# qqueing/DeepSpeaker-pytorch

Measured on AMD Instinct MI355X. Metric: embeddings/sec (64-fbank x 160-frame utterances), higher is better.
Workload: dtype f16

## Files before the change

### deepspeaker-pytorch_amd/_native.py

```python
from __future__ import annotations

import ctypes
import os
from ctypes import POINTER, Structure, c_char_p, c_double, c_float, c_int, c_longlong, c_void_p

_HERE = os.path.dirname(os.path.abspath(__file__))
LIB_NAME = "libdeepspeaker_hip.so"

DS_EPI_AFFINE, DS_EPI_RESIDUAL, DS_EPI_CLIP, DS_EPI_STATS, DS_EPI_OUT_F32, DS_EPI_OUT_F16 = 1, 2, 4, 8, 16, 32
DS_EPI_OUT_PLANES16, DS_CONV_IN_PLANES16 = 256, 512
DS_CONV_HINT_SINGLE_BUFFER = 64
DS_CONV_HINT_CHUNK16 = 128
DS_CONV_HINT_NO_PERSIST = 1024
DS_CONV_HINT_NO_WIDE = 2048
DS_CONV_HINT_ONE_QUEUE = 4096
DS_CONV_PLAN_LATENCY = 8192
DS_CONV_CK = 8
DS_TAIL_SMALL_MAX_B = 4
DS_MARGIN_AAM, DS_MARGIN_AM = 0, 1
DS_MARGIN_SIN2_FLOOR = 1e-6


class ConvShape(Structure):
    _fields_ = [("B", c_int), ("H", c_int), ("W", c_int), ("Cin", c_int),
# ... 19 lines not shown
    "ds_event_elapsed_ms": (c_int, [_P, _P, POINTER(c_float)]),
    "ds_launch_timing_arm": (c_int, [_P, _P]),
    "ds_launch_timing_end": (c_int, []),
    "ds_error_string": (c_char_p, [c_int]),
    "ds_sched_workspace_bytes": (ctypes.c_size_t, []),
    "ds_sched_set_workspace": (c_int, [_P, ctypes.c_size_t]),
    "ds_sched_free_slots": (c_longlong, []),
    "ds_nchw_to_nhwc_f32": (c_int, [_P, _P, c_int, c_int, c_int, c_int, _P]),
    "ds_nhwc_to_nchw_f32": (c_int, [_P, _P, c_int, c_int, c_int, c_int, _P]),
    "ds_pack_conv_weight_f32": (c_int, [_P, _P, c_int, c_int, c_int, c_int, _P]),
    "ds_pack_conv1_weight_f32": (c_int, [_P, _P, c_int, _P]),
    "ds_pack_fc_weight_f32": (c_int, [_P, _P, c_int, c_int, c_int, _P]),
    "ds_pack_fc_weight_dgrad_f32": (c_int, [_P, _P, c_int, c_int, c_int, _P]),
    "ds_bn_fold_f32": (c_int, [_P, _P, _P, _P, c_float, _P, _P, c_int, _P]),
    "ds_bn_stats_finalize_f32": (c_int, [_P, c_int, c_longlong, _P, _P, c_float, c_float, _P, _P, _P, _P,
                                         _P, _P, c_int, _P]),
    "ds_bn_apply_f32": (c_int, [_P, _P, _P, _P, _P, c_longlong, c_int, c_int, _P]),
    "ds_conv_out_dims": (c_int, [POINTER(ConvShape), POINTER(c_int), POINTER(c_int)]),
    "ds_conv_stats_rows": (c_int, [POINTER(ConvShape)]),
    "ds_conv_plan_describe": (c_int, [POINTER(ConvShape), POINTER(c_int)]),
    "ds_conv_f32_set_forced_cfg": (None, [c_int]),
    "ds_conv5x5s2_c1_stats_rows": (c_int, [c_int, c_int]),
    "ds_conv5x5s2_c1_fwd_f32": (c_int, [_P, _P, _P, _P, _P, _P, c_int, c_int, c_int, c_int, c_int, _P]),
    "ds_conv5x5s2_c1_fwd_bf16": (c_int, [_P, _P, _P, _P, _P, _P, c_int, c_int, c_int, c_int, c_int, _P]),
    "ds_conv_fwd_f32": (c_int, [POINTER(ConvShape), _P, _P, _P, _P, _P, _P, _P, c_int, _P]),
    "ds_pack_conv_weight_bf16": (c_int, [_P, _P, _P, c_int, c_int, c_int, _P]),
    "ds_pack_conv_weight_dgrad_bf16": (c_int, [_P, _P, _P, c_int, c_int, c_int, _P]),
    "ds_pack_conv_weight_dgrad_s2_bf16": (c_int, [_P, _P, _P, c_int, c_int, _P]),
    "ds_conv_dgrad_bf16": (c_int, [POINTER(ConvShape), _P, _P, _P, _P, _P]),
    "ds_conv_bf16_stats_rows": (c_int, [POINTER(ConvShape), c_int]),
    "ds_conv_bf16_plan_describe": (c_int, [POINTER(ConvShape), c_int, POINTER(c_int)]),
    "ds_conv_bf16_plan_describe_hinted": (c_int, [POINTER(ConvShape), c_int, c_int, POINTER(c_int)]),
    "ds_conv_bf16_set_forced_cfg": (None, [c_int]),
    "ds_conv_fwd_bf16": (c_int, [POINTER(ConvShape), _P, _P, _P, _P, _P, _P, _P, _P, c_int, _P]),
    "ds_pack_conv_weight_f16": (c_int, [_P, _P, c_int, c_int, c_int, _P]),
    "ds_pack_conv_weights_f16_batch": (c_int, [POINTER(PackJob), c_int, _P]),
    "ds_pack_conv_weights_bf16_batch": (c_int, [POINTER(PackJob), c_int, _P]),
    "ds_conv_fwd_f16": (c_int, [POINTER(ConvShape), _P, _P, _P, _P, _P, _P, c_int, _P]),
    "ds_conv_f16_splitk_workspace_bytes": (c_longlong, [POINTER(ConvShape)]),
    "ds_conv_fwd_f16_splitk": (c_int, [POINTER(ConvShape), _P, _P, _P, _P, _P, _P, c_int, _P, c_longlong, _P]),
    "ds_conv_block_f16_supported": (c_int, [c_int, c_int, c_int, c_int]),
    "ds_conv_block_f16": (c_int, [_P, _P, _P, _P, _P, _P, _P, _P, c_int, c_int, c_int, c_int, c_int, _P]),
    "ds_conv_block_f16_masked": (c_int, [_P, _P, _P, _P, _P, _P, _P, _P, _P, c_int, c_int, c_int, c_int, c_int, _P]),
    "ds_conv_f16_plan_describe": (c_int, [POINTER(ConvShape), POINTER(c_int)]),
    "ds_conv_f16_plan_describe_hinted": (c_int, [POINTER(ConvShape), c_int, POINTER(c_int)]),
    "ds_conv_f16_set_layout_padding": (None, [c_int]),
    "ds_conv_f16_set_forced_cfg": (None, [c_int]),
    "ds_conv_f16_plan_lds_layout": (c_int, [POINTER(ConvShape), c_int, POINTER(c_int)]),
    "ds_cast_f32_to_f16": (c_int, [_P, _P, c_longlong, _P]),
    "ds_cast_f16_to_f32": (c_int, [_P, _P, c_longlong, _P]),
    "ds_avgpool_time_f32": (c_int, [_P, _P, c_int, c_int, c_int, c_int, _P]),
    "ds_l2norm_scale_f32": (c_int, [_P, _P, c_int, c_int, c_float, c_float, _P]),
    "ds_max_abs_diff_f32": (c_int, [_P, _P, c_longlong, _P, _P]),
    "ds_fc_workspace_floats": (c_longlong, [c_int, c_int, c_int]),
    "ds_fc_l2norm_fwd_f32": (c_int, [_P, _P, _P, _P, _P, _P, c_int, c_int, c_int, c_float, c_float, _P]),
    "ds_pairwise_distance_f32": (c_int, [_P, _P, _P, c_int, c_int, _P]),
    "ds_pairwise_distance_p_f32": (c_int, [_P, _P, _P, c_int, c_int, c_float, _P]),
    "ds_pairwise_distance_p_bwd_f32": (c_int, [_P, _P, _P, _P, _P, _P, c_int, c_int, c_float, _P]),
    "ds_triplet_margin_fwd_f32": (c_int, [_P, _P, _P, c_float, _P, _P, _P, c_int, c_int, _P]),
    "ds_triplet_filter_f32": (c_int, [_P, _P, c_float, _P, _P, _P, c_int, _P]),
    "ds_triplet_tail_f32": (c_int, [_P, _P, _P, c_float, c_float, _P, _P, _P, _P, _P, _P, _P, _P, c_int, c_int, c_int, _P]),
    "ds_triplet_scan_f32": (c_int, [_P, _P, c_float, _P, _P, _P, _P, c_int, _P]),
    "ds_refine_distances_f32": (c_int, [_P, _P, _P, c_int, _P, _P, c_int, _P]),
    "ds_triplet_tail_probe_f32": (c_int, [_P, _P, _P, c_float, c_float, _P, _P, _P, _P, _P, _P, _P, _P, c_int, c_int, c_int,
                                          c_int, _P]),
    "ds_refine_distances_probe_f32": (c_int, [_P, _P, _P, c_int, _P, _P, _P, _P, _P, _P, _P, c_int, _P, _P]),
# ... 226 lines not shown
```

### deepspeaker-pytorch_amd/csrc/conv_mfma_bf16.hip

```cpp
#include <ds_device.h>
#include <algorithm>
#include "ds_common.h"

#include "conv_mfma_bf16_kernel.h"
#include "conv_plan.h"

namespace {

__device__ __forceinline__ void pack_conv_weight_bf16_body(const float *w, __bf16 *hi, __bf16 *lo, int Cout, int Cin, int KS,
                                                           int dgrad, int block, int n_blocks) {
    const int T = KS * KS;
    const long long n = (long long)Cout * Cin * T;
    const int N = dgrad ? Cin : Cout;
    for (long long i = (long long)block * 256 + threadIdx.x; i < n; i += (long long)n_blocks * 256) {
        const int kk = (int)(i & 15);
        long long r = i >> 4;
        const int nn = (int)(r % N);
        r /= N;
        const int t = (int)(r % T);
        const int kc = (int)(r / T);
        const int k = kc * 16 + kk;
        const int tt = dgrad ? (T - 1 - t) : t;
        const int kh = tt / KS, kw = tt - kh * KS;
        const int co = dgrad ? k : nn, ci = dgrad ? nn : k;
// ... 18 lines not shown
};

__global__ void __launch_bounds__(256) pack_conv_weight_bf16_batch_kernel(const PackBatchB J) {
    int j = 0;
    while (j + 1 < J.n && (int)blockIdx.x >= J.first[j + 1]) ++j;
    pack_conv_weight_bf16_body(J.w[j], J.hi[j], J.lo[j], J.Cout[j], J.Cin[j], J.KS[j], J.dgrad[j], (int)blockIdx.x - J.first[j],
                               J.first[j + 1] - J.first[j]);
}

static double frag_read_cost(int MT, int NI, int RT, int Wc, int IS, int rows_in, int pitch) {
    const int pix_per_seg = RT * Wc, seg_pix = rows_in * pitch;
    double total = 0.0;
    int n = 0;
    for (int m0 = 0; m0 + 32 <= MT; m0 += 32) {
        for (int g = 0; g < 2; ++g) {
            int cnt[16] = {0};
            int worst = 0;
            for (int j = 0; j < 16; ++j) {
                const int m = m0 + 16 * g + j;
                const int seg = m / pix_per_seg, rem = m % pix_per_seg;
                const int r = rem / Wc, c = rem % Wc;
                const int rec = (seg < NI) ? seg * seg_pix + (IS * r) * pitch + c : 0;
                const int slot = (rec * (PSB / 16)) & 15;
                if (++cnt[slot] > worst) worst = cnt[slot];
            }
            total += worst;
            ++n;
        }
    }
    return n ? total / n : 1.0;
}

static int g_forced_cfg_b = -1;

constexpr int kPlanLatRows = 1;
constexpr int kPlanLatency = 2;

constexpr size_t kLdsSlackB = 16;
static size_t plan_lds_bytes(const TileCfgB &cf, size_t tile_pix, bool x3, int NI) {
    return std::max(tile_pix * PSB * (x3 ? 2 : 1), cf.epi_bytes()) + (size_t)cf.MT() * 4 + (size_t)NI * 8 + (size_t)cf.WM * cf.NTILE() * 8;
}

static int plan_bf16(PlanB &pl, const ds_conv_shape *s, bool x3, int out_stride = 1, int out_h0 = 0, int out_w0 = 0,
                     int out_H = 0, int out_W = 0, int grid_H = 0, int grid_W = 0, int mode = 0) {
    int Ho, Wo;
    const int rc = ds_plan_check_shape(s, CKB, false, Ho, Wo, grid_H, grid_W);
    if (rc != DS_OK) return rc;
    const int pad = s->KS / 2;
    const int yH = out_H > 0 ? out_H : Ho, yW = out_W > 0 ? out_W : Wo;
    DS_REQUIRE((long long)s->B * Ho < (1ll << 24), DS_ERR_BAD_SHAPE);
    DS_REQUIRE((long long)s->B * yH * yW * s->Cout < (1ll << 30), DS_ERR_BAD_SHAPE);
    const int IS = s->stride;
    double best = -1.0;
    int bc = -1, brt = 0, bni = 0;
    long long bwaves = 0, bcost = 0, bblocks = 0;
    bool latency = false;
    auto search = [&](int c) {
        const TileCfgB &cf = ds_bf16_cfg(c);
        if (s->Cout % cf.NTILE()) return;
        if (cf.x3_only && !x3) return;
        if (g_forced_cfg_b >= 0 && c != g_forced_cfg_b) return;
        const long long item_cap = (long long)cf.items_per_thread * cf.NTHR();
        auto fits = [&](int n, int rows_in, int cols_in) {
            return plan_lds_bytes(cf, (size_t)n * rows_in * (cols_in + 4), x3, n) <= cf.lds_cap &&
                   (long long)n * std::min(rows_in, s->H) * s->W * (CKB / 4) <= item_cap;
        };
        ds_plan_segmentations(s->B, Ho, Wo, cf.MT(), IS, s->KS, s->KS, fits, [&](int rt, int ni, long long n_mt) {
            const long long blocks = n_mt * (s->Cout / cf.NTILE());
            double eff = ds_plan_fill_occupancy(s->B, Ho, Wo, n_mt, cf.MT(), blocks, cf.wg_per_cu);
            const long long waves = blocks * (cf.NTHR() / 64);
            if (waves < kPlanSIMDs) eff *= (double)waves / (double)kPlanSIMDs;
            int pref[kNumCfgBAll] = {0, 2, 7, 8, 5, 6, 1, 4, 3, 0, 0};
#ifdef DS_BF16_PREF_TOP
            pref[DS_BF16_PREF_TOP] = 9;
#endif
            eff += 1e-9 * rt + 1e-6 * pref[c];
            bool better = eff > best;
            const long long cost = ds_ceil_div_ll(waves, kPlanSIMDs) * ((x3 ? 3 : 1) * cf.MSUB * cf.NSUB);
            if (latency && bc >= 0) {
                const TileCfgB &bf = ds_bf16_cfg(bc);
                const int area = cf.MT() * cf.NTILE(), barea = bf.MT() * bf.NTILE();
                if (cost != bcost) better = cost < bcost;
                else if (area != barea) better = area > barea;
                else if (blocks != bblocks) better = blocks < bblocks;
            }
            if (better) { best = eff; bc = c; brt = rt; bni = ni; bwaves = waves; bcost = cost; bblocks = blocks; }
        });
    };
    const bool forced_lat = (mode & kPlanLatRows) && g_forced_cfg_b >= kNumCfgB;
    for (int c = 0; c < (forced_lat ? kNumCfgBAll : kNumCfgB); ++c) search(c);
    if ((mode & kPlanLatency) && x3 && g_forced_cfg_b < 0 && bc >= 0 && bwaves < kPlanSIMDs) {
        latency = true;
        best = -1.0;
        bc = -1;
        for (int c = 0; c < kNumCfgBAll; ++c) search(c);
    }
    if (bc < 0) return DS_ERR_UNSUPPORTED;
    const TileCfgB &cf = ds_bf16_cfg(bc);
    ConvKB &k = pl.k;
    k.H = s->H; k.W = s->W; k.Cin = s->Cin;
    k.Hr = Ho; k.Wc = Wo; k.Ho = yH; k.Wo = yW; k.Cout = s->Cout;
    k.OS = out_stride; k.OH0 = out_h0; k.OW0 = out_w0;
    k.IS = IS; k.dh_min = -pad; k.dw_min = -pad;
    pl.cfg = bc;
    ds_plan_fill_geometry(pl, s->B, Ho, Wo, IS, s->KS, s->KS, s->Cout, cf.NTILE(), brt, bni);
    k.half = (k.cols_in + 1) / 2;
    int best_pitch = k.cols_in;
    double best_cost = 1e30;
    for (int pt = k.cols_in; pt <= k.cols_in + 4; ++pt) {
        const double c = frag_read_cost(cf.MT(), bni, brt, Wo, IS, k.rows_in, pt);
        if (c < best_cost - 1e-9) { best_cost = c; best_pitch = pt; }
    }
    k.pitch = best_pitch;
    k.seg_pix = k.rows_in * k.pitch;
    k.y_bytes = (unsigned)((long long)s->B * yH * yW * s->Cout * 4);
    pl.lds_bytes = plan_lds_bytes(cf, (size_t)k.NI * k.seg_pix, x3, k.NI) + kLdsSlackB;
    pl.nit = ds_ceil_div(k.NI * std::min(k.rows_in, s->H) * s->W * (CKB / 4), cf.NTHR());
    k.bn_z = k.bn_mean = k.bn_invstd = k.bn_msc = k.bn_msh = nullptr;
    k.bn_mtiles = 1; k.bn_rows_member = 0; k.bn_row0 = 0;
    return DS_OK;
}

static void set_operands(ConvKB &k, const float *x, const void *w_hi, const void *w_lo, float *y, const float *scale,
                         const float *shift, const float *res, float *stats, int flags) {
    k.x = x; k.w_hi = (const __bf16 *)w_hi; k.w_lo = (const __bf16 *)w_lo; k.y = y;
    k.scale = scale; k.shift = shift; k.res = res; k.stats = stats;
    k.flags = flags;
}

template <int KS, bool X3>
static void launch_b(const PlanB &pl, void *stream) {
    if (pl.cfg >= kNumCfgB) {
        if (KS == 3) ds_bf16_launch_k3x3l(pl, stream); else ds_bf16_launch_k5x3l(pl, stream);
        return;
    }
    if (KS == 3) { if (X3) ds_bf16_launch_k3x3(pl, stream); else ds_bf16_launch_k3x1(pl, stream); }
    else         { if (X3) ds_bf16_launch_k5x3(pl, stream); else ds_bf16_launch_k5x1(pl, stream); }
}

}

static int pack_job_check(const void *w_oihw, const void *w_hi, int Cout, int Cin, int KS, int dgrad, int bad_ks, long long *n) {
    DS_REQUIRE(w_oihw && w_hi, DS_ERR_NULL);
    DS_REQUIRE((dgrad == 0 || dgrad == 1) && Cout > 0 && Cin > 0, DS_ERR_BAD_SHAPE);
    DS_REQUIRE(KS == 3 || KS == 5, bad_ks);
    DS_REQUIRE((dgrad ? Cout : Cin) % CKB == 0, DS_ERR_BAD_SHAPE);
    *n = (long long)Cout * Cin * KS * KS;
    return DS_OK;
}

static int pack_bf16(const float *w_oihw, void *w_hi, void *w_lo, int Cout, int Cin, int KS, int dgrad, void *stream) {
    long long n;
    const int rc = pack_job_check(w_oihw, w_hi, Cout, Cin, KS, dgrad, DS_ERR_BAD_SHAPE, &n);
    if (rc != DS_OK) return rc;
    long long g = (n + 255) / 256;
    DS_LAUNCH(pack_conv_weight_bf16_kernel, (int)(g > 4096 ? 4096 : g), 256, 0, stream, w_oihw, (__bf16 *)w_hi,
              (__bf16 *)w_lo, Cout, Cin, KS, dgrad);
    return ds_last_launch_error();
}

extern "C" int ds_pack_conv_weights_bf16_batch(const ds_pack_job *jobs, int n_jobs, void *stream) {
    DS_REQUIRE(jobs != nullptr, DS_ERR_NULL);
    DS_REQUIRE(n_jobs > 0 && n_jobs <= DS_PACK_BATCH_MAX, DS_ERR_BAD_SHAPE);
    PackBatchB J;
// ... 4 lines not shown
        long long n;
        const int rc = pack_job_check(b.w_oihw, b.out, b.Cout, b.Cin, b.KS, b.mode, DS_ERR_UNSUPPORTED, &n);
        if (rc != DS_OK) return rc;
        J.w[j] = b.w_oihw; J.hi[j] = (__bf16 *)b.out; J.lo[j] = (__bf16 *)b.out2;
        J.Cout[j] = b.Cout; J.Cin[j] = b.Cin; J.KS[j] = b.KS; J.dgrad[j] = b.mode;
        const long long g = (n + 255) / 256;
        J.first[j] = blocks;
        blocks += (int)(g > 512 ? 512 : g);
    }
    J.first[n_jobs] = blocks;
    DS_LAUNCH(pack_conv_weight_bf16_batch_kernel, blocks, 256, 0, stream, J);
    return ds_last_launch_error();
}

extern "C" int ds_pack_conv_weight_bf16(const float *w_oihw, void *w_hi, void *w_lo, int Cout, int Cin, int KS,
                                        void *stream) {
    return pack_bf16(w_oihw, w_hi, w_lo, Cout, Cin, KS, 0, stream);
}

extern "C" int ds_pack_conv_weight_dgrad_bf16(const float *w_oihw, void *w_hi, void *w_lo, int Cout, int Cin, int KS,
                                              void *stream) {
    return pack_bf16(w_oihw, w_hi, w_lo, Cout, Cin, KS, 1, stream);
}

static int fwd_plan_mode(int flags) { return kPlanLatRows | ((flags & DS_CONV_PLAN_LATENCY) ? kPlanLatency : 0); }

extern "C" int ds_conv_bf16_stats_rows(const ds_conv_shape *s, int x3) {
    PlanB pl;
    int rc = plan_bf16(pl, s, x3 != 0, 1, 0, 0, 0, 0, 0, 0, fwd_plan_mode(0));
    return rc == DS_OK ? pl.n_mtiles : rc;
}

extern "C" void ds_conv_bf16_set_forced_cfg(int cfg) { g_forced_cfg_b = (cfg >= 0 && cfg < kNumCfgBAll) ? cfg : -1; }

extern "C" int ds_conv_bf16_plan_describe(const ds_conv_shape *s, int x3, int *out8) {
    return ds_conv_bf16_plan_describe_hinted(s, x3, 0, out8);
}

extern "C" int ds_conv_bf16_plan_describe_hinted(const ds_conv_shape *s, int x3, int flags, int *out8) {
    DS_REQUIRE(out8 != nullptr, DS_ERR_NULL);
    PlanB pl;
    int rc = plan_bf16(pl, s, x3 != 0, 1, 0, 0, 0, 0, 0, 0, fwd_plan_mode(flags));
    if (rc != DS_OK) return rc;
    const TileCfgB &cf = ds_bf16_cfg(pl.cfg);
    out8[0] = cf.MT(); out8[1] = cf.NTILE(); out8[2] = pl.k.RT; out8[3] = pl.k.NI;
    out8[4] = pl.grid; out8[5] = (int)pl.lds_bytes; out8[6] = cf.NTHR(); out8[7] = pl.k.pitch;
    return DS_OK;
}

extern "C" int ds_conv_fwd_bf16(const ds_conv_shape *s, const float *x, const void *w_hi, const void *w_lo,
                                const float *scale, const float *shift, const float *residual, float *y,
                                float *stats_partial, int flags, void *stream) {
    DS_REQUIRE(x && w_hi && y, DS_ERR_NULL);
    DS_REQUIRE(!(flags & DS_EPI_AFFINE) || (scale && shift), DS_ERR_NULL);
    DS_REQUIRE(!(flags & DS_EPI_RESIDUAL) || residual, DS_ERR_NULL);
    DS_REQUIRE(!(flags & DS_EPI_STATS) || stats_partial, DS_ERR_NULL);
    DS_REQUIRE(!((flags & DS_CONV_PLAN_LATENCY) && (flags & DS_EPI_STATS)), DS_ERR_UNSUPPORTED);
    DS_REQUIRE(DS_ALIGNED16(x) && DS_ALIGNED16(w_hi) && DS_ALIGNED16(y) && DS_ALIGNED16(w_lo), DS_ERR_ALIGNMENT);
    const bool x3 = w_lo != nullptr;
    PlanB pl;
    int rc = plan_bf16(pl, s, x3, 1, 0, 0, 0, 0, 0, 0, fwd_plan_mode(flags));
    if (rc != DS_OK) return rc;
    set_operands(pl.k, x, w_hi, w_lo, y, scale, shift, residual, stats_partial, flags & ~DS_CONV_PLAN_LATENCY);
    if (s->KS == 3) { if (x3) launch_b<3, true>(pl, stream); else launch_b<3, false>(pl, stream); }
    else            { if (x3) launch_b<5, true>(pl, stream); else launch_b<5, false>(pl, stream); }
    return ds_last_launch_error();
// ... 176 lines not shown
```

### deepspeaker-pytorch_amd/csrc/conv_mfma_bf16_kernel.h

```cpp
#pragma once
#include <ds_device.h>
#include <type_traits>
#include "ds_common.h"
#include "conv_mfma_f16_parts.h"


constexpr int CKB = 16;
constexpr int PSB = 48;


struct ConvKB {
    const float *x;
    const __bf16 *w_hi, *w_lo;
    float *y;
    const float *scale, *shift, *res;
    float *stats;
    int H, W, Cin;
    int Hr, Wc, Ho, Wo, Cout;
    int IS;
    int dh_min, dw_min;
    int rows_in, cols_in, seg_pix;
    int pitch, half;
    int RT, NI, segs_per_img, n_segs;
    int n_ntiles;
    int flags;
    unsigned y_bytes;
    int OS, OH0, OW0;
    const float *bn_z, *bn_mean, *bn_invstd, *bn_msc, *bn_msh;
    int bn_mtiles;
    int bn_rows_member, bn_row0;
};

struct PlanB {
    int cfg, grid, n_mtiles, nit;
    size_t lds_bytes;
    ConvKB k;
};

struct TileCfgB {
    int MSUB, NSUB, WM, WN;
    int wg_per_cu;
    size_t lds_cap;
    int items_per_thread;
    bool x3_only;
    constexpr int MT() const { return MSUB * WM * 32; }
    constexpr int NTILE() const { return NSUB * WN * 32; }
    constexpr int NTHR() const { return WM * WN * 64; }
    constexpr size_t epi_bytes() const { return (size_t)WM * WN * 32 * (NSUB * 32 + 4) * 4; }
};
constexpr int kNumCfgB = 9;
constexpr TileCfgB kCfgB[kNumCfgB] = {
    {2, 1, 2, 2, 3, 64 * 1024, 16, false},
    {5, 1, 1, 4, 2, 64 * 1024, 16, false},
    {4, 1, 2, 2, 2, 64 * 1024, 16, false},
    {5, 2, 1, 2, 2, 80 * 1024, 32, true},
    {5, 2, 1, 4, 1, 160 * 1024 - 64, 32, true},
    {5, 2, 2, 2, 1, 160 * 1024 - 64, 32, true},
    {5, 2, 2, 1, 2, 80 * 1024, 32, true},
    {4, 2, 1, 2, 2, 80 * 1024, 32, true},
    {4, 2, 1, 4, 1, 160 * 1024 - 64, 32, true},
};

constexpr int kNumCfgBLat = 2;
constexpr TileCfgB kCfgBLat[kNumCfgBLat] = {
    {1, 1, 2, 2, 2, 64 * 1024, 16, true},
    {1, 1, 1, 4, 2, 64 * 1024, 16, true},
};
constexpr int kNumCfgBAll = kNumCfgB + kNumCfgBLat;
constexpr const TileCfgB &ds_bf16_cfg(int cfg) { return cfg < kNumCfgB ? kCfgB[cfg] : kCfgBLat[cfg - kNumCfgB]; }

void ds_bf16_launch_k3x3(const PlanB &pl, void *stream);
void ds_bf16_launch_k5x3(const PlanB &pl, void *stream);
void ds_bf16_launch_k3x1(const PlanB &pl, void *stream);
void ds_bf16_launch_k5x1(const PlanB &pl, void *stream);
void ds_bf16_launch_k3x3g(const PlanB &pl, void *stream);
void ds_bf16_launch_k3x3l(const PlanB &pl, void *stream);
void ds_bf16_launch_k5x3l(const PlanB &pl, void *stream);

#ifdef DS_BF16_KERNEL_TU
namespace {

template <int KS, int MSUB, int NSUB, int WM, int WN, bool X3, int NIT, bool PREF, bool BNB = false>
__global__ void __launch_bounds__(WM * WN * 64) conv_mfma_bf16_kernel(const ConvKB p) {
    constexpr int NTHR = WM * WN * 64;
    constexpr int MT = MSUB * WM * 32;
    constexpr int NTILE = NSUB * WN * 32;
    constexpr int NT = KS * KS;
    constexpr int RING = (KS == 3) ? (MSUB <= 2 ? 9 : 3) : (KS == 5 ? 5 : 1);
    constexpr bool APREF = (MSUB * NSUB >= 8);
    constexpr bool ILV = X3 && APREF;

    char *lds = (char *)ds_dynamic_lds();
    const int tid = threadIdx.x, lane = tid & 63, wave = tid >> 6;
    const int wm = wave / WN, wn = wave % WN;
    const int l31 = lane & 31, lhi = lane >> 5;
    const int tile_n = blockIdx.x % p.n_ntiles;
    const int tile_m = blockIdx.x / p.n_ntiles;
    const int seg0 = tile_m * p.NI;
    const int pix_per_seg = p.RT * p.Wc;
    const int tile_pix = p.NI * p.seg_pix;
    constexpr int EPI_BYTES = WM * WN * 32 * (NSUB * 32 + 4) * 4;
    const int tile_bytes = (X3 ? 2 : 1) * tile_pix * PSB;
    const int stage_bytes = tile_bytes > EPI_BYTES ? tile_bytes : EPI_BYTES;
    char *lds_hi = lds;
    char *lds_lo = lds + (X3 ? tile_pix * PSB : 0);
    int *out_off = (int *)(lds + stage_bytes);
    int *seg_lo = out_off + MT;
    int *seg_cnt = seg_lo + p.NI;
    float *red = (float *)(seg_cnt + p.NI);

    const int n_chunks = p.Cin / CKB;
    const int n_base = tile_n * NTILE + wn * NSUB * 32;
    const size_t lane_w = ((size_t)(n_base + l31) * CKB + 8 * lhi);
    const size_t w_tap_stride = (size_t)p.Cout * CKB;
    const int last_tap = n_chunks * NT - 1;

    bf16x8 bq_hi[RING][NSUB], bq_lo[X3 ? RING : 1][NSUB];
#pragma unroll
    for (int d = 0; d < RING; ++d)
#pragma unroll
        for (int ns = 0; ns < NSUB; ++ns) {
            const int g = d < last_tap ? d : last_tap;
            const size_t o = lane_w + (size_t)g * w_tap_stride + (size_t)ns * 32 * CKB;
            bq_hi[d][ns] = *(const bf16x8 *)(p.w_hi + o);
            if constexpr (X3) bq_lo[d][ns] = *(const bf16x8 *)(p.w_lo + o);
        }

    const float rcp_pps = 1.0f / (float)pix_per_seg, rcp_wc = 1.0f / (float)p.Wc, rcp_w = 1.0f / (float)p.W,
                rcp_spi = 1.0f / (float)p.segs_per_img;
    for (int seg = tid; seg < p.NI; seg += NTHR) {
        const int gseg = seg0 + seg;
        int lo = 0, cnt = 0;
        if (gseg < p.n_segs) {
            const int b = ds_div_small(gseg, p.segs_per_img, rcp_spi);
            const int h0 = p.IS * (gseg - b * p.segs_per_img) * p.RT + p.dh_min;
            lo = h0 < 0 ? -h0 : 0;
// ... 28 lines not shown
                cnt = seg_cnt[seg];
                lo = seg_lo[seg];
                const int gseg = seg0 + seg;
                const int b = ds_div_small(gseg, p.segs_per_img, rcp_spi);
                img_row = b * p.H + p.IS * (gseg - b * p.segs_per_img) * p.RT + p.dh_min;
            }
        };
        next_seg();
#pragma unroll
        for (int it = 0; it < NIT; ++it) {
            while (seg < p.NI && vr >= row0 + cnt) next_seg();
            g_off[it] = 0;
            l_off[it] = 32;
            if (seg < p.NI) {
                const int rr = lo + vr - row0;
                const int cc = c - p.dw_min;
                const int pc = (p.IS == 2) ? ((cc & 1) ? p.half + (cc >> 1) : (cc >> 1)) : cc;
                g_off[it] = ((img_row + rr) * p.W + c) * p.Cin + q * 4;
                l_off[it] = (seg * p.seg_pix + rr * p.pitch + pc) * PSB + q * 8;
            }
            c += dc;
            vr += dvr;
            if (c >= p.W) {
                c -= p.W;
                ++vr;
            }
        }
    }
    f32x4 st[NIT];
    if constexpr (PREF) {
#pragma unroll
        for (int it = 0; it < NIT; ++it) st[it] = *(const f32x4 *)(p.x + g_off[it]);
    }
    for (int i = tid; i < tile_bytes / 16; i += NTHR) *(f32x4 *)(lds + 16 * i) = f32x4{0.0f, 0.0f, 0.0f, 0.0f};
    for (int m = tid; m < MT; m += NTHR) {
        const int seg = ds_div_small(m, pix_per_seg, rcp_pps);
        const int rem = m - seg * pix_per_seg;
        const int r = ds_div_small(rem, p.Wc, rcp_wc), c = rem - r * p.Wc;
        const int gseg = seg0 + seg;
        int off = -1;
        if (seg < p.NI && gseg < p.n_segs) {
            const int b = ds_div_small(gseg, p.segs_per_img, rcp_spi);
            const int rr = (gseg - b * p.segs_per_img) * p.RT + r;
            if (rr < p.Hr) off = ((b * p.Ho + p.OS * rr + p.OH0) * p.Wo + p.OS * c + p.OW0) * p.Cout;
        }
        out_off[m] = off;
    }
    const int lpix = ds_mfma_lpix(l31);
    int a_off[MSUB];
#pragma unroll
    for (int ms = 0; ms < MSUB; ++ms) {
        const int m = (wm * MSUB + ms) * 32 + lpix;
        const int seg = ds_div_small(m, pix_per_seg, rcp_pps);
        const int rem = m - seg * pix_per_seg;
        const int r = ds_div_small(rem, p.Wc, rcp_wc), c = rem - r * p.Wc;
        const int pix = (seg < p.NI) ? seg * p.seg_pix + (p.IS * r) * p.pitch + c : 0;
        a_off[ms] = pix * PSB + 16 * lhi;
    }

    constexpr bool CVI = ILV && PREF;
    constexpr int CV_FIRST = 3;
    auto split_item = [&](int it) {
        const f32x4 v = st[it];
        bf16x8 pk;
#pragma unroll
        for (int j = 0; j < 4; ++j) {
            const __bf16 h = (__bf16)v[j];
            pk[j] = h;
            pk[4 + j] = (__bf16)(v[j] - (float)h);
        }
        st[it] = __builtin_bit_cast(f32x4, pk);
    };
    if constexpr (CVI) {
#pragma unroll
        for (int it = 0; it < NIT; ++it) split_item(it);
    }

    for (int chunk = 0; chunk < n_chunks; ++chunk) {
        __syncthreads();
        if constexpr (!PREF) {
#pragma unroll
            for (int it = 0; it < NIT; ++it) st[it] = *(const f32x4 *)(p.x + g_off[it] + chunk * CKB);
        }
        if constexpr (CVI) {
#pragma unroll
            for (int it = 0; it < NIT; ++it) {
                const bf16x8 pk = __builtin_bit_cast(bf16x8, st[it]);
                *(bf16x4 *)(lds_hi + l_off[it]) = __builtin_shufflevector(pk, pk, 0, 1, 2, 3);
                *(bf16x4 *)(lds_lo + l_off[it]) = __builtin_shufflevector(pk, pk, 4, 5, 6, 7);
            }
        } else {
#pragma unroll
            for (int it = 0; it < NIT; ++it) {
                const f32x4 v = st[it];
                bf16x4 h;
#pragma unroll
                for (int j = 0; j < 4; ++j) h[j] = (__bf16)v[j];
                *(bf16x4 *)(lds_hi + l_off[it]) = h;
                if constexpr (X3) {
                    bf16x4 l;
#pragma unroll
                    for (int j = 0; j < 4; ++j) l[j] = (__bf16)(v[j] - (float)h[j]);
                    *(bf16x4 *)(lds_lo + l_off[it]) = l;
                }
            }
        }
        __syncthreads();
        if constexpr (PREF) {
            const int cn = chunk + 1 < n_chunks ? chunk + 1 : chunk;
#pragma unroll
// ... 271 lines not shown
    else if (pl.nit <= 16)
        DS_LAUNCH_BIG_LDS((conv_mfma_bf16_kernel<KS, MSUB, NSUB, WM, WN, true, 16, true, BNB>), pl.grid, NTHR, pl.lds_bytes, stream, pl.k);
    else
        DS_LAUNCH_BIG_LDS((conv_mfma_bf16_kernel<KS, MSUB, NSUB, WM, WN, true, 32, false, BNB>), pl.grid, NTHR, pl.lds_bytes, stream, pl.k);
}

template <int N = 0, class F>
static void ds_bf16_with_cfg(int cfg, F &&f) {
    if constexpr (N < kNumCfgB) {
        if (cfg == N) f(std::integral_constant<int, N>{});
        else ds_bf16_with_cfg<N + 1>(cfg, f);
    }
}

template <int KS, bool X3, bool BNB = false>
static void launch_b(const PlanB &pl, void *stream) {
    ds_bf16_with_cfg(pl.cfg, [&](auto c) {
        constexpr TileCfgB cf = kCfgB[decltype(c)::value];
        if constexpr (!cf.x3_only) launch_nit_b<KS, cf.MSUB, cf.NSUB, cf.WM, cf.WN, X3, BNB>(pl, stream);
        else if constexpr (X3) launch_big_b<KS, cf.MSUB, cf.NSUB, cf.WM, cf.WN, BNB>(pl, stream);
    });
}

template <int KS, int N = 0>
static void launch_lat_b(const PlanB &pl, void *stream) {
    if constexpr (N < kNumCfgBLat) {
        constexpr TileCfgB cf = kCfgBLat[N];
        static_assert(cf.NTHR() == 256, "launch_nit_b launches 256 threads");
        if (pl.cfg - kNumCfgB == N) launch_nit_b<KS, cf.MSUB, cf.NSUB, cf.WM, cf.WN, true>(pl, stream);
        else launch_lat_b<KS, N + 1>(pl, stream);
    }
}

}
#endif
```

### include/deepspeaker_hip.h

```cpp
#ifndef DEEPSPEAKER_HIP_H
#define DEEPSPEAKER_HIP_H

#include <stddef.h>
#include <stdint.h>

#ifdef __cplusplus
extern "C" {
#endif

#define DS_OK               0
#define DS_ERR_BAD_SHAPE   (-1)
#define DS_ERR_ALIGNMENT   (-2)
#define DS_ERR_NULL        (-3)
#define DS_ERR_UNSUPPORTED (-4)
#define DS_ERR_NO_WORKSPACE (-5)

#define DS_EPI_AFFINE   1
#define DS_EPI_RESIDUAL 2
#define DS_EPI_CLIP     4
#define DS_EPI_STATS    8

#define DS_EPI_OUT_F32  16
#define DS_EPI_OUT_F16  32

// ... 54 lines not shown
    int B, H, W, Cin;
    int Cout, KS;
    int stride;
} ds_conv_shape;

int ds_conv_out_dims(const ds_conv_shape *s, int *Ho, int *Wo);
int ds_conv_stats_rows(const ds_conv_shape *s);

int ds_conv_plan_describe(const ds_conv_shape *s, int *out8);
void ds_conv_f32_set_forced_cfg(int cfg);
int ds_conv5x5s2_c1_stats_rows(int B, int H);
int ds_conv5x5s2_c1_fwd_f32(const float *x, const float *w_packed, const float *scale,
                            const float *shift, float *y, float *stats_partial, int B, int H,
                            int W, int Cout, int flags, void *stream);
int ds_conv5x5s2_c1_fwd_bf16(const float *x, const float *w_packed, const float *scale,
                             const float *shift, void *y, float *stats_partial, int B, int H,
                             int W, int Cout, int flags, void *stream);
int ds_conv_fwd_f32(const ds_conv_shape *s, const float *x, const float *w_packed,
                    const float *scale, const float *shift, const float *residual, float *y,
                    float *stats_partial, int flags, void *stream);

int ds_pack_conv_weight_bf16(const float *w_oihw, void *w_hi, void *w_lo, int Cout, int Cin, int KS,
                             void *stream);
int ds_pack_conv_weight_dgrad_bf16(const float *w_oihw, void *w_hi, void *w_lo, int Cout, int Cin,
                                   int KS, void *stream);
int ds_pack_conv_weight_dgrad_s2_bf16(const float *w_oihw, void *w_hi, void *w_lo, int Cout, int Cin,
                                      void *stream);
int ds_conv_dgrad_bf16(const ds_conv_shape *s, const float *gy, const void *w_hi, const void *w_lo,
                       float *gx, void *stream);
int ds_conv_bf16_stats_rows(const ds_conv_shape *s, int x3);
int ds_conv_bf16_plan_describe(const ds_conv_shape *s, int x3, int *out8);
int ds_conv_bf16_plan_describe_hinted(const ds_conv_shape *s, int x3, int flags, int *out8);
void ds_conv_bf16_set_forced_cfg(int cfg);
int ds_conv_fwd_bf16(const ds_conv_shape *s, const float *x, const void *w_hi, const void *w_lo,
                     const float *scale, const float *shift, const float *residual, float *y,
                     float *stats_partial, int flags, void *stream);

int ds_pack_conv_weight_f16(const float *w_oihw, void *w_f16, int Cout, int Cin, int KS, void *stream);
int ds_conv_fwd_f16(const ds_conv_shape *s, const void *x_f16, const void *w_f16, const float *scale,
                    const float *shift, const void *residual_f16, void *y, int flags, void *stream);
long long ds_conv_f16_splitk_workspace_bytes(const ds_conv_shape *s);
int ds_conv_fwd_f16_splitk(const ds_conv_shape *s, const void *x_f16, const void *w_f16, const float *scale,
                           const float *shift, const void *residual_f16, void *y, int flags, void *workspace,
                           long long ws_bytes, void *stream);
int ds_conv_f16_plan_describe(const ds_conv_shape *s, int *out8);
int ds_conv_f16_plan_describe_hinted(const ds_conv_shape *s, int flags, int *out8);
int ds_conv_f16_plan_lds_layout(const ds_conv_shape *s, int flags, int *out4);
void ds_conv_f16_set_layout_padding(int on);
void ds_conv_f16_set_forced_cfg(int cfg);
int ds_conv_block_f16_supported(int B, int H, int W, int C);
int ds_conv_block_f16(const void *x_f16, const void *wa_f16, const void *wb_f16, const float *scale_a,
                      const float *shift_a, const float *scale_b, const float *shift_b, void *y, int B, int H, int W,
                      int C, int flags, void *stream);
int ds_conv_block_f16_masked(const void *x_f16, const void *wa_f16, const void *wb_f16, const float *scale_a,
                             const float *shift_a, const float *scale_b, const float *shift_b, void *y, const int *lens,
                             int B, int H, int W, int C, int flags, void *stream);
int ds_cast_f32_to_f16(const float *x, void *y_f16, long long n, void *stream);
int ds_cast_f16_to_f32(const void *x_f16, float *y, long long n, void *stream);

int ds_avgpool_time_f32(const float *x, float *pooled, int B, int Hr, int Wc, int C, void *stream);
int ds_l2norm_scale_f32(const float *f, float *e, int B, int D, float alpha, float eps,
                        void *stream);

int ds_max_abs_diff_f32(const float *a, const float *b, long long n, float *out2, void *stream);

long long ds_fc_workspace_floats(int B, int K, int N);
// ... 257 lines not shown
```

Before: 401,200.

## Add double-buffered pipelined bf16x3 conv walk for sub-chip latency plans

Adds a PIPE variant of the bf16x3 MFMA conv kernel that double-buffers the input tile in LDS and interleaves the global load and hi/lo split of the next chunk with the MFMAs of the current chunk. Weight fragments are prefetched through a ring. The planner picks this path for latency-mode x3 plans that occupy less than the chip, when the doubled LDS still fits. The cost is double LDS per block and more template instantiations. This only touches the bf16 x3 path, while the workload is f16 inference, so it likely does not run in the benchmark.

```diff
diff --git a/deepspeaker-pytorch_amd/_native.py b/deepspeaker-pytorch_amd/_native.py
--- a/deepspeaker-pytorch_amd/_native.py
+++ b/deepspeaker-pytorch_amd/_native.py
@@ -75,6 +75,8 @@
     "ds_conv_bf16_plan_describe": (c_int, [POINTER(ConvShape), c_int, POINTER(c_int)]),
     "ds_conv_bf16_plan_describe_hinted": (c_int, [POINTER(ConvShape), c_int, c_int, POINTER(c_int)]),
     "ds_conv_bf16_set_forced_cfg": (None, [c_int]),
+    "ds_conv_bf16_set_walk": (None, [c_int]),
+    "ds_conv_bf16_plan_walk": (c_int, [POINTER(ConvShape), c_int, c_int]),
     "ds_conv_fwd_bf16": (c_int, [POINTER(ConvShape), _P, _P, _P, _P, _P, _P, _P, _P, c_int, _P]),
     "ds_pack_conv_weight_f16": (c_int, [_P, _P, c_int, c_int, c_int, _P]),
     "ds_pack_conv_weights_f16_batch": (c_int, [POINTER(PackJob), c_int, _P]),
diff --git a/deepspeaker-pytorch_amd/csrc/conv_mfma_bf16.hip b/deepspeaker-pytorch_amd/csrc/conv_mfma_bf16.hip
--- a/deepspeaker-pytorch_amd/csrc/conv_mfma_bf16.hip
+++ b/deepspeaker-pytorch_amd/csrc/conv_mfma_bf16.hip
@@ -74,13 +74,15 @@
 }
 
 static int g_forced_cfg_b = -1;
+static int g_walk_b = 0;
 
 constexpr int kPlanLatRows = 1;
 constexpr int kPlanLatency = 2;
 
 constexpr size_t kLdsSlackB = 16;
-static size_t plan_lds_bytes(const TileCfgB &cf, size_t tile_pix, bool x3, int NI) {
-    return std::max(tile_pix * PSB * (x3 ? 2 : 1), cf.epi_bytes()) + (size_t)cf.MT() * 4 + (size_t)NI * 8 + (size_t)cf.WM * cf.NTILE() * 8;
+static size_t plan_lds_bytes(const TileCfgB &cf, size_t tile_pix, bool x3, int NI, bool pipe = false) {
+    return std::max(tile_pix * PSB * (x3 ? 2 : 1) * (pipe ? 2 : 1), cf.epi_bytes()) + (size_t)cf.MT() * 4 + (size_t)NI * 8 +
+           (size_t)cf.WM * cf.NTILE() * 8;
 }
 
 static int plan_bf16(PlanB &pl, const ds_conv_shape *s, bool x3, int out_stride = 1, int out_h0 = 0, int out_w0 = 0,
@@ -131,7 +133,8 @@
     };
     const bool forced_lat = (mode & kPlanLatRows) && g_forced_cfg_b >= kNumCfgB;
     for (int c = 0; c < (forced_lat ? kNumCfgBAll : kNumCfgB); ++c) search(c);
-    if ((mode & kPlanLatency) && x3 && g_forced_cfg_b < 0 && bc >= 0 && bwaves < kPlanSIMDs) {
+    const bool sub_chip = (mode & kPlanLatency) && x3 && bc >= 0 && bwaves < kPlanSIMDs;
+    if (sub_chip && g_forced_cfg_b < 0) {
         latency = true;
         best = -1.0;
         bc = -1;
@@ -156,7 +159,13 @@
     k.pitch = best_pitch;
     k.seg_pix = k.rows_in * k.pitch;
     k.y_bytes = (unsigned)((long long)s->B * yH * yW * s->Cout * 4);
-    pl.lds_bytes = plan_lds_bytes(cf, (size_t)k.NI * k.seg_pix, x3, k.NI) + kLdsSlackB;
+    pl.pipe = 0;
+    if (x3 && (mode & kPlanLatRows) && (g_walk_b == 2 || (g_walk_b == 0 && sub_chip))) {
+        const bool can = ds_bf16_has_pipe(bc) && plan_lds_bytes(cf, (size_t)k.NI * k.seg_pix, true, k.NI, true) + kLdsSlackB <= kLdsCapPipeB;
+        if (!can && g_walk_b == 2) return DS_ERR_UNSUPPORTED;
+        pl.pipe = can;
+    }
+    pl.lds_bytes = plan_lds_bytes(cf, (size_t)k.NI * k.seg_pix, x3, k.NI, pl.pipe != 0) + kLdsSlackB;
     pl.nit = ds_ceil_div(k.NI * std::min(k.rows_in, s->H) * s->W * (CKB / 4), cf.NTHR());
     k.bn_z = k.bn_mean = k.bn_invstd = k.bn_msc = k.bn_msh = nullptr;
     k.bn_mtiles = 1; k.bn_rows_member = 0; k.bn_row0 = 0;
@@ -172,6 +181,10 @@
 
 template <int KS, bool X3>
 static void launch_b(const PlanB &pl, void *stream) {
+    if (pl.pipe) {
+        if (KS == 3) ds_bf16_launch_k3x3p(pl, stream); else ds_bf16_launch_k5x3p(pl, stream);
+        return;
+    }
     if (pl.cfg >= kNumCfgB) {
         if (KS == 3) ds_bf16_launch_k3x3l(pl, stream); else ds_bf16_launch_k5x3l(pl, stream);
         return;
@@ -242,6 +255,14 @@
 }
 
 extern "C" void ds_conv_bf16_set_forced_cfg(int cfg) { g_forced_cfg_b = (cfg >= 0 && cfg < kNumCfgBAll) ? cfg : -1; }
+
+extern "C" void ds_conv_bf16_set_walk(int walk) { g_walk_b = (walk == 1 || walk == 2) ? walk : 0; }
+
+extern "C" int ds_conv_bf16_plan_walk(const ds_conv_shape *s, int x3, int flags) {
+    PlanB pl;
+    const int rc = plan_bf16(pl, s, x3 != 0, 1, 0, 0, 0, 0, 0, 0, fwd_plan_mode(flags));
+    return rc == DS_OK ? (pl.pipe ? 2 : 1) : rc;
+}
 
 extern "C" int ds_conv_bf16_plan_describe(const ds_conv_shape *s, int x3, int *out8) {
     return ds_conv_bf16_plan_describe_hinted(s, x3, 0, out8);
diff --git a/deepspeaker-pytorch_amd/csrc/conv_mfma_bf16_k3x3p.hip b/deepspeaker-pytorch_amd/csrc/conv_mfma_bf16_k3x3p.hip
--- /dev/null
+++ b/deepspeaker-pytorch_amd/csrc/conv_mfma_bf16_k3x3p.hip
@@ -0,0 +1,4 @@
+#define DS_BF16_KERNEL_TU
+#include "conv_mfma_bf16_kernel.h"
+
+void ds_bf16_launch_k3x3p(const PlanB &pl, void *stream) { launch_pipe_b<3>(pl, stream); }
diff --git a/deepspeaker-pytorch_amd/csrc/conv_mfma_bf16_k5x3p.hip b/deepspeaker-pytorch_amd/csrc/conv_mfma_bf16_k5x3p.hip
--- /dev/null
+++ b/deepspeaker-pytorch_amd/csrc/conv_mfma_bf16_k5x3p.hip
@@ -0,0 +1,4 @@
+#define DS_BF16_KERNEL_TU
+#include "conv_mfma_bf16_kernel.h"
+
+void ds_bf16_launch_k5x3p(const PlanB &pl, void *stream) { launch_pipe_b<5>(pl, stream); }
diff --git a/deepspeaker-pytorch_amd/csrc/conv_mfma_bf16_kernel.h b/deepspeaker-pytorch_amd/csrc/conv_mfma_bf16_kernel.h
--- a/deepspeaker-pytorch_amd/csrc/conv_mfma_bf16_kernel.h
+++ b/deepspeaker-pytorch_amd/csrc/conv_mfma_bf16_kernel.h
@@ -33,6 +33,7 @@
 
 struct PlanB {
     int cfg, grid, n_mtiles, nit;
+    int pipe;
     size_t lds_bytes;
     ConvKB k;
 };
@@ -69,6 +70,9 @@
 constexpr int kNumCfgBAll = kNumCfgB + kNumCfgBLat;
 constexpr const TileCfgB &ds_bf16_cfg(int cfg) { return cfg < kNumCfgB ? kCfgB[cfg] : kCfgBLat[cfg - kNumCfgB]; }
 
+constexpr bool ds_bf16_has_pipe(int cfg) { return cfg == 0 || (cfg >= kNumCfgB && cfg < kNumCfgBAll); }
+constexpr size_t kLdsCapPipeB = 160 * 1024 - 64;
+
 void ds_bf16_launch_k3x3(const PlanB &pl, void *stream);
 void ds_bf16_launch_k5x3(const PlanB &pl, void *stream);
 void ds_bf16_launch_k3x1(const PlanB &pl, void *stream);
@@ -76,17 +80,19 @@
 void ds_bf16_launch_k3x3g(const PlanB &pl, void *stream);
 void ds_bf16_launch_k3x3l(const PlanB &pl, void *stream);
 void ds_bf16_launch_k5x3l(const PlanB &pl, void *stream);
+void ds_bf16_launch_k3x3p(const PlanB &pl, void *stream);
+void ds_bf16_launch_k5x3p(const PlanB &pl, void *stream);
 
 #ifdef DS_BF16_KERNEL_TU
 namespace {
 
-template <int KS, int MSUB, int NSUB, int WM, int WN, bool X3, int NIT, bool PREF, bool BNB = false>
+template <int KS, int MSUB, int NSUB, int WM, int WN, bool X3, int NIT, bool PREF, bool BNB = false, bool PIPE = false>
 __global__ void __launch_bounds__(WM * WN * 64) conv_mfma_bf16_kernel(const ConvKB p) {
     constexpr int NTHR = WM * WN * 64;
     constexpr int MT = MSUB * WM * 32;
     constexpr int NTILE = NSUB * WN * 32;
     constexpr int NT = KS * KS;
-    constexpr int RING = (KS == 3) ? (MSUB <= 2 ? 9 : 3) : (KS == 5 ? 5 : 1);
+    constexpr int RING = (KS == 3) ? (MSUB <= 2 ? 9 : 3) : (KS == 5 ? ((PIPE && MSUB * NSUB == 1) ? 25 : 5) : 1);
     constexpr bool APREF = (MSUB * NSUB >= 8);
     constexpr bool ILV = X3 && APREF;
 
@@ -101,7 +107,8 @@
     const int tile_pix = p.NI * p.seg_pix;
     constexpr int EPI_BYTES = WM * WN * 32 * (NSUB * 32 + 4) * 4;
     const int tile_bytes = (X3 ? 2 : 1) * tile_pix * PSB;
-    const int stage_bytes = tile_bytes > EPI_BYTES ? tile_bytes : EPI_BYTES;
+    const int tiles_bytes = (PIPE ? 2 : 1) * tile_bytes;
+    const int stage_bytes = tiles_bytes > EPI_BYTES ? tiles_bytes : EPI_BYTES;
     char *lds_hi = lds;
     char *lds_lo = lds + (X3 ? tile_pix * PSB : 0);
     int *out_off = (int *)(lds + stage_bytes);
@@ -196,7 +203,7 @@
 #pragma unroll
         for (int it = 0; it < NIT; ++it) st[it] = *(const f32x4 *)(p.x + g_off[it]);
     }
-    for (int i = tid; i < tile_bytes / 16; i += NTHR) *(f32x4 *)(lds + 16 * i) = f32x4{0.0f, 0.0f, 0.0f, 0.0f};
+    for (int i = tid; i < tiles_bytes / 16; i += NTHR) *(f32x4 *)(lds + 16 * i) = f32x4{0.0f, 0.0f, 0.0f, 0.0f};
     for (int m = tid; m < MT; m += NTHR) {
         const int seg = ds_div_small(m, pix_per_seg, rcp_pps);
         const int rem = m - seg * pix_per_seg;
@@ -240,6 +247,89 @@
         for (int it = 0; it < NIT; ++it) split_item(it);
     }
 
+    if constexpr (PIPE) {
+        static_assert(X3 && PREF && !BNB && MSUB * NSUB <= 2 && NT % RING == 0, "the pipelined walk: bf16x3, small register tiles");
+        constexpr int NM = 3 * MSUB * NSUB, NR = 2 * NSUB;
+        const int plane = tile_pix * PSB;
+        auto tap_off = [&](int tt) {
+            const int kw = tt % KS;
+            return ((tt / KS) * p.pitch + (p.IS == 2 ? (kw & 1) * p.half + (kw >> 1) : kw)) * PSB;
+        };
+        auto put_item = [&](int it, char *buf, int cn) {
+            const f32x4 v = st[it];
+            bf16x4 h, l;
+#pragma unroll
+            for (int j = 0; j < 4; ++j) {
+                h[j] = (__bf16)v[j];
+                l[j] = (__bf16)(v[j] - (float)h[j]);
+            }
+            *(bf16x4 *)(buf + l_off[it]) = h;
+            *(bf16x4 *)(buf + plane + l_off[it]) = l;
+            st[it] = *(const f32x4 *)(p.x + g_off[it] + cn * CKB);
+        };
+        __syncthreads();
+#pragma unroll
+        for (int it = 0; it < NIT; ++it) put_item(it, lds, n_chunks > 1 ? 1 : 0);
+        __syncthreads();
+        for (int chunk = 0; chunk < n_chunks; ++chunk) {
+            const int rd = (chunk & 1) * tile_bytes;
+            char *wr = lds + (tile_bytes - rd);
+            const int cn = chunk + 2 < n_chunks ? chunk + 2 : n_chunks - 1;
+            const int g0 = chunk * NT;
+            const char *a_cur[MSUB];
+            bf16x8 a_hi[2][MSUB], a_lo[2][MSUB];
+#pragma unroll
+            for (int ms = 0; ms < MSUB; ++ms) {
+                a_cur[ms] = lds + rd + a_off[ms];
+                a_lo[0][ms] = *(const bf16x8 *)(a_cur[ms] + plane + tap_off(0));
+                a_hi[0][ms] = *(const bf16x8 *)(a_cur[ms] + tap_off(0));
+            }
+#pragma unroll
+            for (int t = 0; t < NT; ++t) {
+                const int slot = t % RING, cur = t & 1, rslot = (t + RING - 1) % RING;
+                __builtin_amdgcn_sched_barrier(0);
+                if (t + 1 < NT) {
+                    const int toff = tap_off(t + 1);
+#pragma unroll
+                    for (int ms = 0; ms < MSUB; ++ms) a_lo[cur ^ 1][ms] = *(const bf16x8 *)(a_cur[ms] + plane + toff);
+#pragma unroll
+                    for (int ms = 0; ms < MSUB; ++ms) a_hi[cur ^ 1][ms] = *(const bf16x8 *)(a_cur[ms] + toff);
+                }
+                int gn = g0 + t - 1 + RING;
+                gn = gn < last_tap ? gn : last_tap;
+                const __bf16 *rhi = p.w_hi + lane_w + (size_t)gn * w_tap_stride;
+                const __bf16 *rlo = p.w_lo + lane_w + (size_t)gn * w_tap_stride;
+                const int i0 = (NIT * t) / NT, i1 = (NIT * (t + 1)) / NT;
+                __builtin_amdgcn_sched_barrier(0);
+#pragma unroll
+                for (int q = 0; q < NM; ++q) {
+                    const int term = q / (MSUB * NSUB), ms = (q % (MSUB * NSUB)) / NSUB, ns = q % NSUB;
+                    if (term == 0) acc[ms][ns] = ds_mfma_32x32x16_bf16(bq_hi[slot][ns], a_lo[cur][ms], acc[ms][ns]);
+                    else if (term == 1) acc[ms][ns] = ds_mfma_32x32x16_bf16(bq_lo[slot][ns], a_hi[cur][ms], acc[ms][ns]);
+                    else acc[ms][ns] = ds_mfma_32x32x16_bf16(bq_hi[slot][ns], a_hi[cur][ms], acc[ms][ns]);
+                    if (t > 0 && q < NR) {
+                        if (q & 1) bq_lo[rslot][q >> 1] = *(const bf16x8 *)(rlo + (size_t)(q >> 1) * 32 * CKB);
+                        else bq_hi[rslot][q >> 1] = *(const bf16x8 *)(rhi + (size_t)(q >> 1) * 32 * CKB);
+                    }
+#pragma unroll
+                    for (int it = i0; it < i1; ++it)
+                        if (NR + (it - i0) % (NM - NR) == q) put_item(it, wr, cn);
+                    __builtin_amdgcn_sched_barrier(0);
+                }
+            }
+            {
+                int gn = g0 + NT - 1 + RING;
+                gn = gn < last_tap ? gn : last_tap;
+#pragma unroll
+                for (int ns = 0; ns < NSUB; ++ns) {
+                    const size_t o = lane_w + (size_t)gn * w_tap_stride + (size_t)ns * 32 * CKB;
+                    bq_hi[(NT - 1) % RING][ns] = *(const bf16x8 *)(p.w_hi + o);
+                    bq_lo[(NT - 1) % RING][ns] = *(const bf16x8 *)(p.w_lo + o);
+                }
+            }
+            ds_lds_barrier();
+        }
+    } else
     for (int chunk = 0; chunk < n_chunks; ++chunk) {
         __syncthreads();
         if constexpr (!PREF) {
@@ -577,5 +667,25 @@
     }
 }
 
+template <int KS, int MSUB, int NSUB, int WM, int WN>
+static void launch_pipe_nit_b(const PlanB &pl, void *stream) {
+    static_assert(WM * WN * 64 == 256, "256 threads");
+    if (pl.nit <= 4)
+        DS_LAUNCH_BIG_LDS((conv_mfma_bf16_kernel<KS, MSUB, NSUB, WM, WN, true, 4, true, false, true>), pl.grid, 256, pl.lds_bytes, stream, pl.k);
+    else if (pl.nit <= 8)
+        DS_LAUNCH_BIG_LDS((conv_mfma_bf16_kernel<KS, MSUB, NSUB, WM, WN, true, 8, true, false, true>), pl.grid, 256, pl.lds_bytes, stream, pl.k);
+    else
+        DS_LAUNCH_BIG_LDS((conv_mfma_bf16_kernel<KS, MSUB, NSUB, WM, WN, true, 16, true, false, true>), pl.grid, 256, pl.lds_bytes, stream, pl.k);
+}
+
+template <int KS>
+static void launch_pipe_b(const PlanB &pl, void *stream) {
+    constexpr TileCfgB c0 = kCfgB[0], l0 = kCfgBLat[0], l1 = kCfgBLat[1];
+    static_assert(kNumCfgBLat == 2 && ds_bf16_has_pipe(0) && ds_bf16_has_pipe(kNumCfgB) && ds_bf16_has_pipe(kNumCfgB + 1), "");
+    if (pl.cfg == 0) launch_pipe_nit_b<KS, c0.MSUB, c0.NSUB, c0.WM, c0.WN>(pl, stream);
+    else if (pl.cfg == kNumCfgB) launch_pipe_nit_b<KS, l0.MSUB, l0.NSUB, l0.WM, l0.WN>(pl, stream);
+    else if (pl.cfg == kNumCfgB + 1) launch_pipe_nit_b<KS, l1.MSUB, l1.NSUB, l1.WM, l1.WN>(pl, stream);
+}
+
 }
 #endif
diff --git a/include/deepspeaker_hip.h b/include/deepspeaker_hip.h
--- a/include/deepspeaker_hip.h
+++ b/include/deepspeaker_hip.h
@@ -110,6 +110,8 @@
 int ds_conv_bf16_plan_describe(const ds_conv_shape *s, int x3, int *out8);
 int ds_conv_bf16_plan_describe_hinted(const ds_conv_shape *s, int x3, int flags, int *out8);
 void ds_conv_bf16_set_forced_cfg(int cfg);
+void ds_conv_bf16_set_walk(int walk);
+int ds_conv_bf16_plan_walk(const ds_conv_shape *s, int x3, int flags);
 int ds_conv_fwd_bf16(const ds_conv_shape *s, const float *x, const void *w_hi, const void *w_lo,
                      const float *scale, const float *shift, const float *residual, float *y,
                      float *stats_partial, int flags, void *stream);
```

After: 405,800 (median of 6 runs). 1.01x the previous value.
